# hszhao/semseg

Measured on NVIDIA H100. Metric: PSPNet50 473x473 training images/sec, higher is better.
Workload: dtype bf16

## Files before the change

include/semseg_b200.h:

```cpp
#ifndef SEMSEG_B200_H
#define SEMSEG_B200_H

#include <stdint.h>

#ifdef __cplusplus
extern "C" {
#endif

#define SEMSEG_OK 0
#define SEMSEG_E_INVALID (-1)
#define SEMSEG_E_CUDA (-2)
#define SEMSEG_E_UNSUPPORTED (-3)

#define SEMSEG_MAX_TAPS 9

const char* semseg_last_error(void);
int semseg_abi_version(void);
long long semseg_launch_count(void);

int semseg_psamask_fwd(int psa_type, const float* in, float* out, int N, int H, int W, int mH, int mW,
                       void* stream);
int semseg_psamask_bwd(int psa_type, const float* dout, float* din, int N, int H, int W, int mH, int mW,
                       void* stream);

// ... 46 lines not shown
  void* y_lo;
  const void* residual_lo;
  int32_t w_split;
  int32_t k_slices;
  int64_t slice_stride;
} semseg_conv_desc;

int semseg_conv_k_slices(int Cin, int taps, int max_kblocks);
int semseg_conv_splitk_rows(int M);
int semseg_conv_splitk_finish(const float* partial, int k_slices, long long slice_stride, int part_pitch, int M, int C,
                              int epi_mode, int relu, const float* scale, const float* shift, const void* residual,
                              const void* residual_lo, int res_pitch, void* y, void* y_lo, int y_pitch,
                              float* stats_partial, void* stream);
int semseg_conv_stats_rows(int N, int H, int W, int Cout);
int semseg_conv_fprop(const semseg_conv_desc* d, void* stream);

typedef struct semseg_wgrad_desc {
  int32_t N, H, W;
  int32_t Cin, Cout;
  const void* x;
  int32_t Nin, Hin, Win, x_pitch;
  const void* dy;
  int32_t dy_pitch;
  int32_t taps;
  int32_t dh[SEMSEG_MAX_TAPS], dw[SEMSEG_MAX_TAPS];
  int32_t img_mul, img_add[SEMSEG_MAX_TAPS];
  float* dw_partial;
  int32_t n_splits;
  const void* x_lo;
  const void* dy_lo;
} semseg_wgrad_desc;

int semseg_conv_wgrad_splits(const semseg_wgrad_desc* d);
int semseg_conv_wgrad(const semseg_wgrad_desc* d, void* stream);
int semseg_wgrad_reduce(const float* dw_partial, int n_splits, int taps, int Cout, int Cin, float* dw_oihw,
                        int accumulate, void* stream);

typedef struct semseg_pack_item {
  const float* w;
  void* wf;
  void* wd;
  void* wp;
  int Cout, Cin, taps;
  int cols_f, cols_d;
  int tile0, tiles_ci;
  int split;
} semseg_pack_item;
int semseg_pack_weights_multi(const semseg_pack_item* items_dev, int n_items, int n_tiles, int max_taps, void* stream);

// ... 267 lines not shown
```

semseg_b200/_lib.py:

```python
import ctypes
import os

_HERE = os.path.dirname(os.path.abspath(__file__))
LIB_PATH = os.path.join(_HERE, "lib", "libsemseg_b200.so")

MAX_TAPS = 9
EPI_RAW, EPI_AFFINE, EPI_F32 = 0, 1, 2
PSA_DENSE, PSA_NO_SOFTMAX = 1, 2

c_int = ctypes.c_int
c_i32 = ctypes.c_int32
c_vp = ctypes.c_void_p
c_f = ctypes.c_float
c_ll = ctypes.c_longlong
I9 = c_i32 * MAX_TAPS


class PackItem(ctypes.Structure):
    _fields_ = [
        ("w", c_vp), ("wf", c_vp), ("wd", c_vp), ("wp", c_vp),
        ("Cout", c_i32), ("Cin", c_i32), ("taps", c_i32),
        ("cols_f", c_i32), ("cols_d", c_i32),
        ("tile0", c_i32), ("tiles_ci", c_i32),
        ("split", c_i32),
# ... 72 lines not shown
    "semseg_psa_attend": (c_int, [c_int, c_int, c_vp, c_int, c_vp, c_vp, c_int, c_vp, c_vp, c_vp, c_int, c_int, c_int,
                                  c_int, c_int, c_int, c_int, c_f, c_vp]),
    "semseg_psa_attend_bwd_attn": (c_int, [c_int, c_vp, c_int, c_vp, c_vp, c_vp, c_int, c_vp, c_vp, c_int, c_vp, c_vp,
                                           c_int, c_vp, c_int, c_int, c_int, c_int, c_int, c_int, c_f, c_vp]),
    "semseg_psa_attend_ex": (c_int, [c_int, c_int, c_int, c_vp, c_int, c_vp, c_vp, c_int, c_vp, c_vp, c_vp, c_int,
                                     c_int, c_int, c_int, c_int, c_int, c_int, c_f, c_vp]),
    "semseg_psa_attend_bwd_attn_ex": (c_int, [c_int, c_int, c_vp, c_int, c_vp, c_vp, c_vp, c_int, c_vp, c_vp, c_int,
                                              c_vp, c_vp, c_int, c_vp, c_int, c_int, c_int, c_int, c_int, c_int, c_f,
                                              c_vp]),
    "semseg_conv_stats_rows": (c_int, [c_int, c_int, c_int, c_int]),
    "semseg_conv_k_slices": (c_int, [c_int, c_int, c_int]),
    "semseg_conv_splitk_rows": (c_int, [c_int]),
    "semseg_conv_splitk_finish": (c_int, [c_vp, c_int, c_ll, c_int, c_int, c_int, c_int, c_int, c_vp, c_vp, c_vp, c_vp,
                                          c_int, c_vp, c_vp, c_int, c_vp, c_vp]),
    "semseg_conv_fprop": (c_int, [ctypes.POINTER(ConvDesc), c_vp]),
    "semseg_conv_wgrad_splits": (c_int, [ctypes.POINTER(WgradDesc)]),
    "semseg_conv_wgrad": (c_int, [ctypes.POINTER(WgradDesc), c_vp]),
    "semseg_wgrad_reduce": (c_int, [c_vp, c_int, c_int, c_int, c_int, c_vp, c_int, c_vp]),
    "semseg_pack_weights_multi": (c_int, [c_vp, c_int, c_int, c_int, c_vp]),
    "semseg_sgd_chunk_elems": (c_int, []),
    "semseg_sgd_multi": (c_int, [c_vp, c_vp, c_int, c_int, ctypes.POINTER(SgdHyper), c_vp]),
    "semseg_ema_multi": (c_int, [c_vp, c_int, c_int, ctypes.c_double, c_vp]),
    "semseg_iou_hist": (c_int, [c_vp, c_vp, ctypes.c_longlong, c_int, ctypes.c_longlong, c_int, c_vp, c_vp]),
    "semseg_im2col3x3s2": (c_int, [c_vp, c_int, c_int, c_int, c_int, c_int, c_vp, c_vp]),
    "semseg_stem_dgrad3x3s2": (c_int, [c_vp, c_vp, c_int, c_int, c_int, c_int, c_int, c_int, c_int, c_int, c_vp, c_int,
                                       c_vp, c_vp]),
    "semseg_nchw_f32_to_nhwc_bf16": (c_int, [c_vp, c_vp, c_vp, c_int, c_int, c_int, c_int, c_int, c_vp]),
    "semseg_nhwc_bf16_to_nchw_f32": (c_int, [c_vp, c_vp, c_vp, c_int, c_int, c_int, c_int, c_int, c_vp]),
    "semseg_nhwc_f32_to_nchw_f32": (c_int, [c_vp, c_vp, c_int, c_int, c_int, c_int, c_int, c_vp]),
    "semseg_space_to_phases": (c_int, [c_vp, c_int, c_int, c_int, c_int, c_int, c_vp, c_vp]),
    "semseg_phases_to_space": (c_int, [c_vp, c_int, c_int, c_int, c_int, c_vp, c_vp]),
    "semseg_bn_merge_partials": (c_int, [c_vp, c_int, c_int, c_vp, c_vp]),
# ... 152 lines not shown
```

semseg_b200/csrc/conv_igemm.cu:

```cuda
#include "host_common.h"
#include "ptx.cuh"

namespace sb {

constexpr int kBlockM = 128;
constexpr int kBlockK = 64;
constexpr int kConvThreads = 384;
constexpr int kConsumerThreads = 256;
constexpr int kATileBytes = kBlockM * kBlockK * 2;
constexpr int kStageOutBytes = kBlockM * 64 * 2;
constexpr int kMiscBytes = 2048;

template <int BLOCK_N>
struct ConvCfg {
  static constexpr int kBTileBytes = BLOCK_N * kBlockK * 2;
  static constexpr int kStageBytes = kATileBytes + kBTileBytes;
  static constexpr int kStages = (BLOCK_N == 256) ? 4 : (BLOCK_N == 128 ? 6 : 8);
  static constexpr int kSmemBytes = kStages * kStageBytes + 2 * kStageOutBytes + kMiscBytes + 1024;
};

struct ConvKParams {
  int N, H, W;
  int Cin, Cout;
  int taps;
// ... 2 lines not shown
  int k_chunks;
  int dh[SEMSEG_MAX_TAPS], dw[SEMSEG_MAX_TAPS], wtap[SEMSEG_MAX_TAPS], img_add[SEMSEG_MAX_TAPS];
  int img_mul;
  int epi_mode, relu;
  const float* scale;
  const float* shift;
  const __nv_bfloat16* residual;
  const __nv_bfloat16* residual_lo;
  int res_pitch;
  int nseg;
  int k_slices, kb_per_slice;
  long long slice_stride;
  float* out_f32;
  int out_pitch;
  float* stats_partial;
};

template <int BLOCK_N, bool kSplit>
__global__ void __launch_bounds__(kConvThreads, 1)
conv_igemm_kernel(const __grid_constant__ CUtensorMap tmA, const __grid_constant__ CUtensorMap tmB,
                  const __grid_constant__ CUtensorMap tmC, const __grid_constant__ CUtensorMap tmA_lo,
                  const __grid_constant__ CUtensorMap tmB_lo, const __grid_constant__ CUtensorMap tmC_lo,
                  const ConvKParams p) {
  using Cfg = ConvCfg<BLOCK_N>;
  constexpr int kStages = Cfg::kStages;
  constexpr int kStageBytes = Cfg::kStageBytes;
  constexpr int kAcc = BLOCK_N / 2;
  const int num_items = p.num_m_tiles * p.n_tiles * p.k_slices;
  auto decode_item = [&](int item, int& m_tile, int& n_tile, int& k_slice) {
    k_slice = item % p.k_slices;
    item /= p.k_slices;
// ... 5 lines not shown
    const int tiles_per_img = p.tiles_h * p.tiles_w;
    img = m_tile / tiles_per_img;
    const int rem = m_tile - img * tiles_per_img;
    h0 = (rem / p.tiles_w) * p.bh;
    w0 = (rem % p.tiles_w) * p.bw;
  };

  extern __shared__ __align__(1024) uint8_t smem_raw[];
  uint8_t* smem = smem_raw + ((1024u - (smem_u32(smem_raw) & 1023u)) & 1023u);
  uint8_t* stage_base = smem;
  uint8_t* out_stage = smem + kStages * kStageBytes;
  uint8_t* misc = out_stage + 2 * kStageOutBytes;
  static_assert(kStages <= 16, "barrier area sized for <= 16 stages");
  uint64_t* full_bar = reinterpret_cast<uint64_t*>(misc);
  uint64_t* empty_bar = full_bar + 16;

  const int warp = threadIdx.x >> 5;
  const int lane = threadIdx.x & 31;
  const int nseg = kSplit ? p.nseg : 1;
  const int total_kblk = p.taps * p.k_chunks;
  auto slice_range = [&](int k_slice, int& kblk0, int& kblk1) {
    kblk0 = k_slice * p.kb_per_slice;
    kblk1 = min(kblk0 + p.kb_per_slice, total_kblk);
  };
  const uint32_t stage_tx = static_cast<uint32_t>(p.bh * p.bw) * 128u + static_cast<uint32_t>(Cfg::kBTileBytes);

  if (warp == 0 && lane == 0) {
    tma_prefetch_desc(&tmA);
    tma_prefetch_desc(&tmB);
    tma_prefetch_desc(&tmC);
    if (kSplit) {
      tma_prefetch_desc(&tmA_lo);
      tma_prefetch_desc(&tmB_lo);
      tma_prefetch_desc(&tmC_lo);
// ... 2 lines not shown
      mbar_init(&full_bar[i], 1);
      mbar_init(&empty_bar[i], kConsumerThreads);
    }
    fence_barrier_init();
  }
  if (p.stats_partial != nullptr) {
    float* row = p.stats_partial + static_cast<size_t>(blockIdx.x) * 4 * 3 * p.Cout;
    for (int i = threadIdx.x; i < 4 * 3 * p.Cout; i += kConvThreads) row[i] = 0.f;
  }
  __syncthreads();

  if (warp < 4) {
    setmaxnreg_dec<40>();
    if (warp == 0 && elect_one()) {
      int it = 0;
      for (int item = blockIdx.x; item < num_items; item += gridDim.x) {
        int m_tile, n_tile, k_slice, kblk0, kblk1;
        decode_item(item, m_tile, n_tile, k_slice);
        slice_range(k_slice, kblk0, kblk1);
        const int tiles_per_img = p.tiles_h * p.tiles_w;
        const int img = m_tile / tiles_per_img;
        const int rem = m_tile - img * tiles_per_img;
        const int h0 = (rem / p.tiles_w) * p.bh;
        const int w0 = (rem % p.tiles_w) * p.bw;
        const int n0 = n_tile * BLOCK_N;
        for (int kb = kblk0 * nseg; kb < kblk1 * nseg; ++kb, ++it) {
          const int s = it % kStages;
          const uint32_t par = (it / kStages) & 1;
          mbar_wait(&empty_bar[s], par ^ 1);
          const int ks = kb / nseg;
          const int seg = kb - ks * nseg;
          const int cb = ks / p.taps;
          const int t = ks - cb * p.taps;
          const CUtensorMap* mA = (kSplit && seg == 1) ? &tmA_lo : &tmA;
          const CUtensorMap* mB = (kSplit && seg == 2) ? &tmB_lo : &tmB;
          uint8_t* a_dst = stage_base + s * kStageBytes;
          uint8_t* b_dst = a_dst + kATileBytes;
          mbar_expect_tx(&full_bar[s], stage_tx);
          tma_load_4d(a_dst, mA, &full_bar[s], cb * kBlockK, w0 + p.dw[t], h0 + p.dh[t],
                      img * p.img_mul + p.img_add[t]);
          tma_load_3d(b_dst, mB, &full_bar[s], cb * kBlockK, n0, p.wtap[t]);
        }
      }
    }
  } else {
    setmaxnreg_inc<232>();
    const int ct = threadIdx.x - 128;
    const int wg = ct >> 7;
    const int wq = (ct >> 5) & 3;
    const int r_base = wg * 64 + wq * 16 + (lane >> 2);
    const int cq = 2 * (lane & 3);
    int it = 0;
    int store_buf = 0;
    float acc[kAcc];
    constexpr int kChunks = BLOCK_N / 64;
    const bool stats = p.stats_partial != nullptr && p.epi_mode == SEMSEG_EPI_RAW;
    float st_acc[kChunks][2], st_n = 0.f;
#pragma unroll
    for (int ch = 0; ch < kChunks; ++ch) st_acc[ch][0] = st_acc[ch][1] = 0.f;
    for (int item = blockIdx.x; item < num_items; item += gridDim.x) {
      int m_tile, n_tile, k_slice, kblk0, kblk1;
      decode_item(item, m_tile, n_tile, k_slice);
      slice_range(k_slice, kblk0, kblk1);
      const int num_kb = (kblk1 - kblk0) * nseg;
      if (p.epi_mode == SEMSEG_EPI_AFFINE && p.residual != nullptr && (lane & 3) < kChunks) {
        const int c = n_tile * BLOCK_N + 64 * (lane & 3);
        int img, h0, w0;
        tile_origin(m_tile, img, h0, w0);
#pragma unroll
        for (int i = 0; i < 2; ++i) {
          const int r = r_base + 8 * i, hi = r / p.bw, wi = r - hi * p.bw;
          if (c < p.Cout && r < p.bh * p.bw && h0 + hi < p.H && w0 + wi < p.W) {
            const long long ro = ((static_cast<long long>(img) * p.H + (h0 + hi)) * p.W + (w0 + wi)) * p.res_pitch + c;
            prefetch_l2(p.residual + ro);
            if (kSplit) prefetch_l2(p.residual_lo + ro);
// ... 169 lines not shown
            for (int v = 0; v < 3; ++v) old[ch][v] = st_dst[ch * 64 + v * p.Cout];
#pragma unroll
        for (int ch = 0; ch < kChunks; ++ch) {
          if (n0 + ch * 64 < p.Cout) {
            st_dst[ch * 64] = old[ch][0] + st_acc[ch][0];
            st_dst[ch * 64 + p.Cout] = old[ch][1] + st_acc[ch][1];
            st_dst[ch * 64 + 2 * p.Cout] = old[ch][2] + st_n;
          }
          st_acc[ch][0] = st_acc[ch][1] = 0.f;
        }
        st_n = 0.f;
      }
    }
    if (ct == 0) tma_store_wait_all<0>();
  }
}

static int conv_grid(int num_m_tiles, int n_tiles) {
  const int sms = num_sms();
  const long long tiles = static_cast<long long>(num_m_tiles) * n_tiles;
  return static_cast<int>(tiles < sms ? tiles : sms);
}

struct ConvMaps {
  CUtensorMap a, b, c, a_lo, b_lo, c_lo;
};

template <int BLOCK_N>
static int launch_conv(const ConvMaps& tm, const ConvKParams& kp, bool split, int grid, cudaStream_t stream) {
  using Cfg = ConvCfg<BLOCK_N>;
// ... 26 lines not shown

extern "C" int semseg_conv_k_slices(int Cin, int taps, int max_kblocks) {
  if (Cin <= 0 || taps <= 0 || max_kblocks <= 0) return SEMSEG_E_INVALID;
  const int total = taps * sb::cdiv(Cin, sb::kBlockK);
  const int per = sb::cdiv(total, sb::cdiv(total, max_kblocks));
  return sb::cdiv(total, per);
}

extern "C" int semseg_conv_stats_rows(int N, int H, int W, int Cout) {
  if (N <= 0 || H <= 0 || W <= 0 || Cout <= 0) return SEMSEG_E_INVALID;
  int bh, bw;
  sb::choose_box(H, W, sb::kBlockM, &bh, &bw);
  return 4 * sb::conv_grid(N * sb::cdiv(H, bh) * sb::cdiv(W, bw), sb::cdiv(Cout, conv_block_n(Cout)));
}

extern "C" int semseg_conv_fprop(const semseg_conv_desc* d, void* stream_) {
  using namespace sb;
  cudaStream_t stream = static_cast<cudaStream_t>(stream_);
  SB_CHECK_ARG(d != nullptr, "conv: null descriptor");
  SB_CHECK_ARG(d->N > 0 && d->H > 0 && d->W > 0 && d->Cin > 0 && d->Cout > 0, "conv: bad sizes");
  SB_CHECK_ARG(d->taps >= 1 && d->taps <= SEMSEG_MAX_TAPS, "conv: taps=%d out of range", d->taps);
  SB_CHECK_ARG(d->x && d->w, "conv: null x/w");
  SB_CHECK_ARG(d->x_pitch % 8 == 0 && d->x_pitch >= d->Cin, "conv: x_pitch %d must be a multiple of 8 and >= Cin",
               d->x_pitch);
  SB_CHECK_ARG(d->w_cols % 8 == 0 && d->w_cols >= d->Cin, "conv: w_cols %d must be a multiple of 8 and >= Cin",
               d->w_cols);
  SB_CHECK_ARG(d->epi_mode >= 0 && d->epi_mode <= 2, "conv: bad epi_mode");

  ConvKParams kp;
  memset(&kp, 0, sizeof(kp));
  kp.N = d->N; kp.H = d->H; kp.W = d->W; kp.Cin = d->Cin; kp.Cout = d->Cout; kp.taps = d->taps;
  choose_box(d->H, d->W, kBlockM, &kp.bh, &kp.bw);
  kp.tiles_h = cdiv(d->H, kp.bh);
// ... 8 lines not shown
  kp.epi_mode = d->epi_mode; kp.relu = d->relu;
  kp.scale = d->scale; kp.shift = d->shift;
  kp.residual = static_cast<const __nv_bfloat16*>(d->residual); kp.res_pitch = d->res_pitch;
  kp.residual_lo = static_cast<const __nv_bfloat16*>(d->residual_lo);
  const bool split = d->x_lo != nullptr;
  kp.nseg = split ? 3 : 1;
  if (split) {
    SB_CHECK_ARG(d->w_split != 0, "conv: split activations need split weights (w_split)");
    SB_CHECK_ARG(d->epi_mode == SEMSEG_EPI_F32 || d->y_lo != nullptr, "conv: split input needs a split output (y_lo)");
    SB_CHECK_ARG(!d->residual || d->residual_lo, "conv: split input needs a split residual (residual_lo)");
  } else {
    SB_CHECK_ARG(!d->y_lo && !d->residual_lo, "conv: lo planes given without x_lo");
  }
  kp.out_f32 = d->out_f32; kp.out_pitch = d->out_pitch;
  kp.stats_partial = d->stats_partial;

  const int block_n = conv_block_n(d->Cout);
  kp.n_tiles = cdiv(d->Cout, block_n);
  kp.k_slices = 1;
  kp.kb_per_slice = kp.taps * kp.k_chunks;
  kp.slice_stride = 0;
  if (d->k_slices > 1) {
    SB_CHECK_ARG(d->epi_mode == SEMSEG_EPI_F32, "conv: K slicing needs the F32 epilogue (partials are fp32)");
    SB_CHECK_ARG(d->slice_stride >= static_cast<long long>(d->N) * d->H * d->W * d->out_pitch,
                 "conv: slice_stride too small for an [N,H,W,out_pitch] partial");
    kp.kb_per_slice = cdiv(kp.taps * kp.k_chunks, d->k_slices);
    kp.k_slices = cdiv(kp.taps * kp.k_chunks, kp.kb_per_slice);
    SB_CHECK_ARG(kp.k_slices == d->k_slices, "conv: k_slices %d not realisable for %d K blocks (use %d)", d->k_slices,
                 kp.taps * kp.k_chunks, kp.k_slices);
    kp.slice_stride = d->slice_stride;
// ... 39 lines not shown
    uint64_t dims[4] = {(uint64_t)d->Cout, (uint64_t)d->W, (uint64_t)d->H, (uint64_t)d->N};
    uint64_t str[3] = {(uint64_t)d->y_pitch * 2, (uint64_t)d->y_pitch * 2 * d->W,
                       (uint64_t)d->y_pitch * 2 * d->W * d->H};
    uint32_t box[4] = {64u, (uint32_t)kp.bw, (uint32_t)kp.bh, 1};
    int r = encode_tmap_bf16(&tm.c, d->y, 4, dims, str, box);
    if (r) return r;
    tm.c_lo = tm.c;
    if (split && (r = encode_tmap_bf16(&tm.c_lo, d->y_lo, 4, dims, str, box))) return r;
  }
  switch (block_n) {
    case 256: return launch_conv<256>(tm, kp, split, grid, stream);
    case 128: return launch_conv<128>(tm, kp, split, grid, stream);
    default: return launch_conv<64>(tm, kp, split, grid, stream);
  }
}
```

semseg_b200/csrc/conv_wgrad.cu:

```cuda
#include "host_common.h"
#include "ptx.cuh"

namespace sb {

constexpr int kWgThreads = 384;
constexpr int kWgConsumerThreads = 256;
constexpr int kWgBoxPixels = 64;
constexpr int kWgBoxBytes = kWgBoxPixels * 128;
constexpr int kWgABoxes = 2;

template <int BN>
struct WgCfg {
  static constexpr int kBBoxes = BN / 64;
  static constexpr int kStageBytes = (kWgABoxes + kBBoxes) * kWgBoxBytes;
  static constexpr int kStages = BN == 256 ? 4 : (BN == 128 ? 6 : 8);
  static constexpr int kSmemBytes = kStages * kStageBytes + 1024 + 1024;
};

struct WgradKParams {
  int N, H, W, Cin, Cout, taps;
  int bh, bw, tiles_h, tiles_w, num_boxes;
  int co_tiles, ci_tiles, n_splits, boxes_per_split, block_n;
  int tu, cin_boxes, unit_taps, oob_img;
  int dh[SEMSEG_MAX_TAPS], dw[SEMSEG_MAX_TAPS], img_add[SEMSEG_MAX_TAPS];
// ... 293 lines not shown
    }
  }
  kp->boxes_per_split = cdiv(kp->num_boxes, splits);
  kp->n_splits = cdiv(kp->num_boxes, kp->boxes_per_split);
}

}

extern "C" int semseg_conv_wgrad_splits(const semseg_wgrad_desc* d) {
  if (!d || d->N <= 0 || d->H <= 0 || d->W <= 0 || d->Cin <= 0 || d->Cout <= 0) return SEMSEG_E_INVALID;
  sb::WgradKParams kp;
  sb::wgrad_geometry(d, &kp);
  return kp.n_splits;
}

extern "C" int semseg_conv_wgrad(const semseg_wgrad_desc* d, void* stream_) {
  using namespace sb;
  cudaStream_t stream = static_cast<cudaStream_t>(stream_);
  SB_CHECK_ARG(d != nullptr, "wgrad: null descriptor");
  SB_CHECK_ARG(d->N > 0 && d->H > 0 && d->W > 0 && d->Cin > 0 && d->Cout > 0, "wgrad: bad sizes");
  SB_CHECK_ARG(d->taps >= 1 && d->taps <= SEMSEG_MAX_TAPS, "wgrad: taps out of range");
  SB_CHECK_ARG(d->x && d->dy && d->dw_partial, "wgrad: null pointer");
  SB_CHECK_ARG(d->x_pitch % 8 == 0 && d->dy_pitch % 8 == 0, "wgrad: pitches must be multiples of 8");
  WgradKParams kp;
  memset(&kp, 0, sizeof(kp));
  wgrad_geometry(d, &kp);
  if (d->n_splits > 0)
    SB_CHECK_ARG(kp.n_splits == d->n_splits, "wgrad: n_splits %d not realisable (library would use %d)",
                 d->n_splits, kp.n_splits);
  for (int t = 0; t < d->taps; ++t) {
    kp.dh[t] = d->dh[t]; kp.dw[t] = d->dw[t]; kp.img_add[t] = d->img_add[t];
  }
  kp.img_mul = d->img_mul;
// ... 13 lines not shown
    tmDY_lo = tmDY;
    if (split && (r = encode_tmap_bf16(&tmDY_lo, d->dy_lo, 4, dims, str, box))) return r;
  }
  {
    uint64_t dims[4] = {(uint64_t)d->Cin, (uint64_t)d->Win, (uint64_t)d->Hin, (uint64_t)d->Nin};
    uint64_t str[3] = {(uint64_t)d->x_pitch * 2, (uint64_t)d->x_pitch * 2 * d->Win,
                       (uint64_t)d->x_pitch * 2 * d->Win * d->Hin};
    uint32_t box[4] = {64u, (uint32_t)kp.bw, (uint32_t)kp.bh, 1};
    int r = encode_tmap_bf16(&tmX, d->x, 4, dims, str, box);
    if (r) return r;
    tmX_lo = tmX;
    if (split && (r = encode_tmap_bf16(&tmX_lo, d->x_lo, 4, dims, str, box))) return r;
  }
  const int units = kp.unit_taps * kp.co_tiles * kp.ci_tiles * kp.n_splits;
  int rc = SEMSEG_OK;
  const int grid = units < num_sms() ? units : num_sms();
  switch (kp.block_n) {
    case 256: rc = launch_wgrad<256>(tmDY, tmX, tmDY_lo, tmX_lo, kp, grid, stream); break;
    case 128: rc = launch_wgrad<128>(tmDY, tmX, tmDY_lo, tmX_lo, kp, grid, stream); break;
    default: rc = launch_wgrad<64>(tmDY, tmX, tmDY_lo, tmX_lo, kp, grid, stream); break;
  }
  if (rc) return rc;
  SB_LAUNCHED();
  return SEMSEG_OK;
}

extern "C" int semseg_wgrad_reduce(const float* dw_partial, int n_splits, int taps, int Cout, int Cin,
                                   float* dw_oihw, int accumulate, void* stream_) {
  using namespace sb;
  cudaStream_t stream = static_cast<cudaStream_t>(stream_);
  SB_CHECK_ARG(dw_partial && dw_oihw && n_splits > 0 && taps > 0 && Cout > 0 && Cin > 0, "wgrad_reduce: bad args");
  SB_CHECK_ARG(taps <= kRedMaxTaps, "wgrad_reduce: at most 9 taps");
  const size_t plane = static_cast<size_t>(Cout) * Cin;
  const int groups = taps >= 8 ? 1 : 8 / taps;
  const dim3 block(32, taps, groups);
  if (plane % 4 == 0) {
    const size_t per_block = static_cast<size_t>(128) * groups;
    const unsigned blocks = static_cast<unsigned>((plane + per_block - 1) / per_block);
    const size_t smem = static_cast<size_t>(groups) * taps * (128 + 4) * sizeof(float);
// ... 11 lines not shown
```

semseg_b200/functional.py:

```python
import contextlib
import functools
import threading

import torch
import torch.distributed as dist
import torch.nn as nn
import torch.nn.functional as F

from . import losses
from . import ops
from . import p2p
from . import precision
from .dist_utils import gather_rank_stats
from .ops import EPI_RAW, EPI_AFFINE, EPI_F32


def packed(conv, need_dgrad=True, split=False):
    w = conv.weight
    key = (w._version, w.data_ptr(), need_dgrad, split)
    cache = conv.__dict__.get("_sb_pack")
    if cache is not None and cache[0] == key:
        return cache[1]
    if cache is not None and cache[0][:2] == key[:2] and cache[0][3] == split and cache[0][2]:
        return cache[1]
# ... 171 lines not shown
            raise NotImplementedError("semseg_b200: input gradient of a stride-2 conv needs Cin % 64 == 0")
        hh, wh = self.xin.shape[-3], self.xin.shape[-2]
        dxp = ops.empty_act((4 * n, hh, wh, pw.cin), ops.is_split(d_raw), d_raw.device)
        for q in range(4):
            sub = [t for t, a in zip(mirrored, self.img_add) if a == q * n]
            part = ops.act_batch_slice(dxp, q * n, (q + 1) * n)
            if sub:
                ops.conv_fprop(d_raw, pw.wd, pw.cin, sub, out=part, out_nhw=(n, hh, wh))
            else:
                part.zero_()
        dx = ops.phases_to_space(dxp, n, h, w)
        return dx if dx_add is None else ops.add_act(dx, dx_add)

    def wgrad(self, d_raw):
        pw = self.pw
        dw = ops.conv_wgrad(self.xin, d_raw, self.xin.shape[-1], pw.cout, self.taps, img_add=self.img_add)
        if self.kind == "patches":
            return dw[:, :9 * pw.cin, 0, 0].reshape(pw.cout, 3, 3, pw.cin).permute(0, 3, 1, 2).contiguous()
        return dw[:, :pw.cin].contiguous() if dw.shape[1] != pw.cin else dw


class _CbaState:
    __slots__ = ("form", "bn", "frozen", "relu", "has_res", "raw", "y", "mi", "ss", "pg")


def cba_forward(x, conv, bn, relu, residual, out=None, input_needs_grad=True, mode="batch"):
    form = _ConvForm(conv, x, input_needs_grad, mode)
    raw = mi = pg = None
    if mode == "batch":
        raw, sp = form.fprop(stats=True)
        pg = _sync_group(bn)
# ... 17 lines not shown
def cba_backward(st, dy, need_dx=True, need_dw=True, need_dres=False, dx_add=None, dx_nchw=False):
    bn = st.bn
    want_dres = st.has_res and need_dres
    if st.frozen:
        want_g, want_b = st.raw is not None, bn.bias is not None and bn.bias.requires_grad
        if not (need_dx or need_dw or want_dres or want_g or want_b):
            return None, None, None, None, None
        d_raw, dres, sums = ops.bn_bwd_frozen(dy if dy.is_contiguous() else dy.contiguous(), st.y, st.raw, bn.weight,
                                              bn.bias, bn.running_mean, bn.running_var, bn.eps, st.relu,
                                              want_dres=want_dres, want_sums=want_g or want_b)
        dgamma = sums[1] if want_g else None
        dbeta = sums[0] if want_b else None
    else:
        d_raw, dres, dgamma, dbeta = _bn_backward(st.pg, dy, st.y, st.raw, st.mi, bn.weight, st.relu, want_dres, st.ss)
    dx = st.form.dgrad(d_raw, dx_add, nchw=dx_nchw) if need_dx else None
    dw = st.form.wgrad(d_raw) if need_dw else None
    return dx, dw, dgamma, dbeta, dres


class _ConvBnAct(torch.autograd.Function):

    @staticmethod
    def forward(ctx, x, weight, gamma, beta, residual, conv, bn, relu, out, frozen):
        ctx.nchw = x.dtype != torch.bfloat16
        xa = ops.nchw_to_nhwc_bf16(x.contiguous().float(), split=precision.split_enabled()) if ctx.nchw else x
        y, st = cba_forward(xa, conv, bn, relu, residual, out, input_needs_grad=ctx.needs_input_grad[0],
                            mode="frozen" if frozen else "batch")
        ctx.st = st
        if out is not None:
            ctx.mark_dirty(out)
        return y
# ... 105 lines not shown
        ctx.save_for_backward(x)
        ctx.pw = pw
        return y

    @staticmethod
    def backward(ctx, dy):
        (x,) = ctx.saved_tensors
        pw = ctx.pw
        n, h, w, c = dy.shape
        cp = pw.wd.shape[-1]
        dyb = ops.f32_to_act(dy.contiguous(), ops.is_split(x))
        dx = dw = db = None
        if ctx.needs_input_grad[0]:
            dx, _ = ops.conv_fprop(dyb, pw.wd, pw.cin, ops.conv_taps(1, 1))
        if ctx.needs_input_grad[1]:
            dwp = ops.conv_wgrad(x, dyb, pw.cin, cp, ops.conv_taps(1, 1))
            dw = dwp[:c].contiguous()
        if ctx.needs_input_grad[2]:
            db = dy.sum(dim=(0, 1, 2))
        return dx, dw, db, None


def conv_bias_f32(x, conv):
    assert conv.kernel_size == (1, 1) and conv.stride == (1, 1) and x.shape[-1] % 8 == 0
    if torch.is_grad_enabled() and (x.requires_grad or conv.weight.requires_grad):
        return _ConvBiasF32.apply(x, conv.weight, conv.bias, conv)
    pw = packed(conv, need_dgrad=False, split=ops.is_split(x))
    y, _ = ops.conv_fprop(x, pw.wf, pw.cout, ops.conv_taps(1, 1), epi=EPI_F32, shift=conv.bias)
    return y


class _UpsampleCE(torch.autograd.Function):
# ... 524 lines not shown
```

semseg_b200/graphs.py:

```python
import os
import warnings

import torch
import torch.distributed as dist

from . import precision

WARMUP_CALLS = 3
MAX_GRAPHS = 4
_capturing = False
_boundary = None


def enabled():
    return os.environ.get("SEMSEG_B200_GRAPH", "1") != "0"


def capturing():
    return _capturing


def note_boundary(t):
    global _boundary
    if _capturing and t.requires_grad:
        _boundary = t
    return t


class _Step:
    __slots__ = ("key", "calls", "failed", "fwd", "bwd", "bwd2", "x", "y", "pred", "main", "aux", "g_main", "g_aux",
                 "grads", "grads2", "t_mid", "d_mid", "n_tail", "params", "pool", "keep", "launches", "dx_slot", "mix",
                 "mix_crit", "strong", "strong_crit", "fp", "fp_crit")

    def __init__(self, key):
# ... 117 lines not shown
    from . import _lib
    slots, seen = [], set()
    for mod in model.modules():
        for name, prm in mod._parameters.items():
            if prm is not None and prm.requires_grad and id(prm) not in seen:
                seen.add(id(prm))
                slots.append((mod, name, prm))
    st.params = [prm for _, _, prm in slots]
    st.x, st.y = torch.empty_like(x), torch.empty_like(y)
    st.x.copy_(x.detach())
    st.y.copy_(y)
    torch.cuda.synchronize()
    st.pool = torch.cuda.graph_pool_handle()
    st.fwd, st.bwd, st.bwd2 = torch.cuda.CUDAGraph(), torch.cuda.CUDAGraph(), None
    l0 = _lib.launch_count()
    global _boundary
    _capturing, _boundary = True, None
    proxies = []
    st.dx_slot = x.requires_grad
    x_in = st.x.detach().requires_grad_(True) if st.dx_slot else st.x
    x_leaf = [x_in] if st.dx_slot else []
    try:
        for mod, name, prm in slots:
            q = prm.detach().requires_grad_(True)
            mod._parameters[name] = q
            proxies.append(q)
        with torch.cuda.graph(st.fwd, pool=st.pool, capture_error_mode="thread_local"):
            with torch.enable_grad():
                st.pred, st.main, st.aux = impl(x_in, st.y)
        st.g_main, st.g_aux = torch.ones_like(st.main), torch.ones_like(st.aux)
        t_mid = _boundary
        head_ids = set()
        if t_mid is not None and os.environ.get("SEMSEG_B200_GRAPH_SEGMENTS", "2") != "1":
            for name in getattr(model, "_sb_head_modules", ()):
                head_ids.update(id(q) for q in getattr(model, name).parameters() if q.requires_grad)
        if head_ids:
            order = [k for k, q in enumerate(proxies) if id(q) in head_ids] + \
                    [k for k, q in enumerate(proxies) if id(q) not in head_ids]
            n_head = len(head_ids)
            st.params = [st.params[k] for k in order]
            prox_head = [proxies[k] for k in order[:n_head]]
            prox_tail = [proxies[k] for k in order[n_head:]]
            with torch.cuda.graph(st.bwd, pool=st.pool, capture_error_mode="thread_local"):
                gs = torch.autograd.grad((st.main, st.aux), [t_mid] + prox_tail, (st.g_main, st.g_aux), allow_unused=True)
            st.d_mid, st.grads = gs[0], gs[1:]
            st.bwd2 = torch.cuda.CUDAGraph()
            with torch.cuda.graph(st.bwd2, pool=st.pool, capture_error_mode="thread_local"):
                st.grads2 = torch.autograd.grad((t_mid,), prox_head + x_leaf, (st.d_mid,), allow_unused=True)
            st.t_mid, st.n_tail = t_mid.detach(), len(prox_tail)
        else:
            with torch.cuda.graph(st.bwd, pool=st.pool, capture_error_mode="thread_local"):
                st.grads = torch.autograd.grad((st.main, st.aux), proxies + x_leaf, (st.g_main, st.g_aux),
                                               allow_unused=True)
    finally:
        _capturing, _boundary = False, None
        for mod, name, prm in slots:
            mod._parameters[name] = prm
    st.launches = _lib.launch_count() - l0
    crit = getattr(model, "criterion", None)
    if getattr(crit, "_mix_state", None) is not None:
        st.mix, st.mix_crit = crit._mix_state, crit
    if getattr(crit, "strong", None) is not None:
        st.strong, st.strong_crit = crit._strong_state, crit
    if getattr(crit, "fp_weight", 0.0) > 0.0:
        st.fp, st.fp_crit = crit._fp_state, crit
    st.pred, st.main, st.aux = st.pred.detach(), st.main.detach(), st.aux.detach()
    del proxies, x_in, x_leaf
    st.keep = model.__dict__.get("_sb_pack_plan")
    teacher = _teacher(getattr(model, "criterion", None))
    if teacher is not None:
# ... 77 lines not shown
```

semseg_b200/ops.py:

```python
import ctypes

import torch

from . import _lib
from . import p2p
from ._lib import ConvDesc, WgradDesc, EPI_RAW, EPI_AFFINE, EPI_F32, MAX_TAPS


X3_MAX_KBLOCKS = 8

_raw_stream = getattr(torch._C, "_cuda_getCurrentRawStream", None)
_cur_device = getattr(torch._C, "_cuda_getDevice", None)


def _stream():
    if _raw_stream is not None and _cur_device is not None:
        return ctypes.c_void_p(_raw_stream(_cur_device()))
    return ctypes.c_void_p(torch.cuda.current_stream().cuda_stream)


def _ptr(t):
    return ctypes.c_void_p(t.data_ptr()) if t is not None else ctypes.c_void_p(0)


def _require_cuda(*ts):
    for t in ts:
        if t is not None and not t.is_cuda:
            raise _lib.SemsegError("semseg_b200 ops require CUDA tensors (no CPU fallback); got device %s" % t.device)


def is_split(t):
    return t is not None and t.dim() == 5

# ... 278 lines not shown
    if shift is not None:
        assert shift.dtype == torch.float32 and shift.numel() >= cout
        d.shift = shift.data_ptr()
    if residual is not None:
        rn, rh, rw, rc, rp = _nhwc_meta(residual)
        assert (rn, rh, rw, rc) == (n, h, w, cout) and is_split(residual) == split
        d.residual, d.res_pitch, d.residual_lo = residual.data_ptr(), rp, _lo_int(residual)
    k_slices = int(lib.semseg_conv_k_slices(cin, len(taps), X3_MAX_KBLOCKS)) if (split and epi != EPI_F32) else 1
    if k_slices > 1:
        part = torch.empty((k_slices, n, h, w, cout), dtype=torch.float32, device=x.device)
        d.epi_mode, d.relu = EPI_F32, 0
        d.out_f32, d.out_pitch = part.data_ptr(), cout
        d.k_slices, d.slice_stride = k_slices, part.stride(0)
        sc, sh, rs, rsl, rpitch, ylo = d.scale, d.shift, d.residual, d.residual_lo, d.res_pitch, d.y_lo
        d.scale = d.shift = d.residual = d.residual_lo = d.y_lo = None
        _lib.check(lib.semseg_conv_fprop(ctypes.byref(d), _stream()), "semseg_conv_fprop (K-sliced)")
        m = n * h * w
        if stats:
            assert epi == EPI_RAW
            sp = torch.empty((int(lib.semseg_conv_splitk_rows(m)), 3, cout), dtype=torch.float32, device=x.device)
        _lib.check(lib.semseg_conv_splitk_finish(_ptr(part), k_slices, part.stride(0), cout, m, cout, epi,
                                                 int(bool(relu)), sc, sh, rs, rsl, rpitch, d.y, ylo, d.y_pitch,
                                                 _ptr(sp), _stream()), "semseg_conv_splitk_finish")
        return y, sp
    if stats:
        assert epi == EPI_RAW
        sp = torch.empty((conv_stats_rows(n, h, w, cout), 3, cout), dtype=torch.float32, device=x.device)
        d.stats_partial = sp.data_ptr()
    _lib.check(lib.semseg_conv_fprop(ctypes.byref(d), _stream()), "semseg_conv_fprop")
    return y, sp


def conv_wgrad(x, dy, cin, cout, taps, grad_out=None, accumulate=False, img_add=None):
    _require_cuda(x, dy)
    lib = _lib.load()
    nin, hin, win, xc, xp = _nhwc_meta(x)
    n, h, w, dc, dp = _nhwc_meta(dy)
    assert xc >= cin and dc >= cout
    assert img_add is not None or (nin, hin, win) == (n, h, w)
    _same_form(x, dy)
    d = WgradDesc()
    d.N, d.H, d.W, d.Cin, d.Cout = n, h, w, cin, cout
    d.x, d.Nin, d.Hin, d.Win, d.x_pitch = x.data_ptr(), nin, hin, win, xp
    d.dy, d.dy_pitch = dy.data_ptr(), dp
    d.x_lo, d.dy_lo = _lo_int(x), _lo_int(dy)
    _fill_taps(d, taps, with_wtap=False, img_add=img_add)
    d.n_splits = 0
    splits = lib.semseg_conv_wgrad_splits(ctypes.byref(d))
    if splits <= 0:
        raise _lib.SemsegError("semseg_conv_wgrad_splits failed (%d)" % splits)
    ntaps = len(taps)
    part = torch.empty((splits, ntaps, cout, cin), dtype=torch.float32, device=x.device)
    d.dw_partial = part.data_ptr()
    d.n_splits = splits
    _lib.check(lib.semseg_conv_wgrad(ctypes.byref(d), _stream()), "semseg_conv_wgrad")
    k = int(round(ntaps ** 0.5))
    if grad_out is None:
        grad_out = torch.empty((cout, cin, k, k), dtype=torch.float32, device=x.device)
        accumulate = False
    assert grad_out.is_contiguous() and grad_out.dtype == torch.float32
    _lib.check(lib.semseg_wgrad_reduce(_ptr(part), splits, ntaps, cout, cin, _ptr(grad_out), int(accumulate),
                                       _stream()), "semseg_wgrad_reduce")
    return grad_out


def nchw_to_nhwc_bf16(x, pad_to=8, split=False):
    _require_cuda(x)
    lib = _lib.load()
    assert x.dtype == torch.float32 and x.is_contiguous()
    n, c, h, w = x.shape
# ... 872 lines not shown
```

Before: 299.7.

## Overlap weight-gradient convs on a side stream with dynamically scheduled convs

During CUDA-graph capture, weight-gradient convolutions are launched on a side stream with their grid capped to leave SMs free, so they can run concurrently with the data-gradient path on the main stream. The conv fprop kernel gains an optional dynamic tile scheduler. A global atomic counter per stream slot hands out work items, and the producer forwards each item ID to the consumers through shared memory, so CTAs that share the GPU with side-stream work balance their load. This adds atomic traffic, a self-resetting counter that assumes no two concurrent launches share a slot, and stream synchronisation joins at the end of backward.

```diff
diff --git a/include/semseg_b200.h b/include/semseg_b200.h
--- a/include/semseg_b200.h
+++ b/include/semseg_b200.h
@@ -84,6 +84,8 @@
                               float* stats_partial, void* stream);
 int semseg_conv_stats_rows(int N, int H, int W, int Cout);
 int semseg_conv_fprop(const semseg_conv_desc* d, void* stream);
+int semseg_conv_sched_slots(void);
+int semseg_conv_fprop_sched(const semseg_conv_desc* d, int slot, void* stream);
 
 typedef struct semseg_wgrad_desc {
   int32_t N, H, W;
@@ -103,6 +105,7 @@
 
 int semseg_conv_wgrad_splits(const semseg_wgrad_desc* d);
 int semseg_conv_wgrad(const semseg_wgrad_desc* d, void* stream);
+int semseg_conv_wgrad_grid(const semseg_wgrad_desc* d, int max_ctas, void* stream);
 int semseg_wgrad_reduce(const float* dw_partial, int n_splits, int taps, int Cout, int Cin, float* dw_oihw,
                         int accumulate, void* stream);
 
diff --git a/semseg_b200/_lib.py b/semseg_b200/_lib.py
--- a/semseg_b200/_lib.py
+++ b/semseg_b200/_lib.py
@@ -110,8 +110,11 @@
     "semseg_conv_splitk_finish": (c_int, [c_vp, c_int, c_ll, c_int, c_int, c_int, c_int, c_int, c_vp, c_vp, c_vp, c_vp,
                                           c_int, c_vp, c_vp, c_int, c_vp, c_vp]),
     "semseg_conv_fprop": (c_int, [ctypes.POINTER(ConvDesc), c_vp]),
+    "semseg_conv_sched_slots": (c_int, []),
+    "semseg_conv_fprop_sched": (c_int, [ctypes.POINTER(ConvDesc), c_int, c_vp]),
     "semseg_conv_wgrad_splits": (c_int, [ctypes.POINTER(WgradDesc)]),
     "semseg_conv_wgrad": (c_int, [ctypes.POINTER(WgradDesc), c_vp]),
+    "semseg_conv_wgrad_grid": (c_int, [ctypes.POINTER(WgradDesc), c_int, c_vp]),
     "semseg_wgrad_reduce": (c_int, [c_vp, c_int, c_int, c_int, c_int, c_vp, c_int, c_vp]),
     "semseg_pack_weights_multi": (c_int, [c_vp, c_int, c_int, c_int, c_vp]),
     "semseg_sgd_chunk_elems": (c_int, []),
diff --git a/semseg_b200/csrc/conv_igemm.cu b/semseg_b200/csrc/conv_igemm.cu
--- a/semseg_b200/csrc/conv_igemm.cu
+++ b/semseg_b200/csrc/conv_igemm.cu
@@ -40,7 +40,11 @@
   float* out_f32;
   int out_pitch;
   float* stats_partial;
+  unsigned* sched;
 };
+
+constexpr int kSchedSlots = 64;
+__device__ unsigned g_conv_sched[kSchedSlots][2];
 
 template <int BLOCK_N, bool kSplit>
 __global__ void __launch_bounds__(kConvThreads, 1)
@@ -76,10 +80,12 @@
   static_assert(kStages <= 16, "barrier area sized for <= 16 stages");
   uint64_t* full_bar = reinterpret_cast<uint64_t*>(misc);
   uint64_t* empty_bar = full_bar + 16;
+  int* stage_item = reinterpret_cast<int*>(empty_bar + 16);
 
   const int warp = threadIdx.x >> 5;
   const int lane = threadIdx.x & 31;
   const int nseg = kSplit ? p.nseg : 1;
+  const bool dynamic = p.sched != nullptr;
   const int total_kblk = p.taps * p.k_chunks;
   auto slice_range = [&](int k_slice, int& kblk0, int& kblk1) {
     kblk0 = k_slice * p.kb_per_slice;
@@ -112,7 +118,9 @@
     setmaxnreg_dec<40>();
     if (warp == 0 && elect_one()) {
       int it = 0;
-      for (int item = blockIdx.x; item < num_items; item += gridDim.x) {
+      for (int item = dynamic ? static_cast<int>(atomicAdd(&p.sched[0], 1u)) : static_cast<int>(blockIdx.x), next;
+           item < num_items; item = next) {
+        next = dynamic ? static_cast<int>(atomicAdd(&p.sched[0], 1u)) : item + static_cast<int>(gridDim.x);
         int m_tile, n_tile, k_slice, kblk0, kblk1;
         decode_item(item, m_tile, n_tile, k_slice);
         slice_range(k_slice, kblk0, kblk1);
@@ -134,11 +142,18 @@
           const CUtensorMap* mB = (kSplit && seg == 2) ? &tmB_lo : &tmB;
           uint8_t* a_dst = stage_base + s * kStageBytes;
           uint8_t* b_dst = a_dst + kATileBytes;
+          if (dynamic && kb == kblk0 * nseg) stage_item[s] = item;
           mbar_expect_tx(&full_bar[s], stage_tx);
           tma_load_4d(a_dst, mA, &full_bar[s], cb * kBlockK, w0 + p.dw[t], h0 + p.dh[t],
                       img * p.img_mul + p.img_add[t]);
           tma_load_3d(b_dst, mB, &full_bar[s], cb * kBlockK, n0, p.wtap[t]);
         }
+      }
+      if (dynamic) {
+        const int s = it % kStages;
+        mbar_wait(&empty_bar[s], ((it / kStages) & 1) ^ 1);
+        stage_item[s] = num_items;
+        mbar_arrive(&full_bar[s]);
       }
     }
   } else {
@@ -156,7 +171,13 @@
     float st_acc[kChunks][2], st_n = 0.f;
 #pragma unroll
     for (int ch = 0; ch < kChunks; ++ch) st_acc[ch][0] = st_acc[ch][1] = 0.f;
-    for (int item = blockIdx.x; item < num_items; item += gridDim.x) {
+    for (int item = static_cast<int>(blockIdx.x);; item += gridDim.x) {
+      if (dynamic) {
+        const int s = it % kStages;
+        mbar_wait(&full_bar[s], (it / kStages) & 1);
+        item = stage_item[s];
+      }
+      if (item >= num_items) break;
       int m_tile, n_tile, k_slice, kblk0, kblk1;
       decode_item(item, m_tile, n_tile, k_slice);
       slice_range(k_slice, kblk0, kblk1);
@@ -356,6 +377,16 @@
     }
     if (ct == 0) tma_store_wait_all<0>();
   }
+  if (dynamic) {
+    __syncthreads();
+    if (threadIdx.x == 0) {
+      __threadfence();
+      if (atomicAdd(&p.sched[1], 1u) == gridDim.x - 1) {
+        atomicExch(&p.sched[0], 0u);
+        atomicExch(&p.sched[1], 0u);
+      }
+    }
+  }
 }
 
 static int conv_grid(int num_m_tiles, int n_tiles) {
@@ -412,9 +443,10 @@
   return 4 * sb::conv_grid(N * sb::cdiv(H, bh) * sb::cdiv(W, bw), sb::cdiv(Cout, conv_block_n(Cout)));
 }
 
-extern "C" int semseg_conv_fprop(const semseg_conv_desc* d, void* stream_) {
+extern "C" int semseg_conv_sched_slots() { return sb::kSchedSlots; }
+
+static int conv_fprop_launch(const semseg_conv_desc* d, int slot, cudaStream_t stream) {
   using namespace sb;
-  cudaStream_t stream = static_cast<cudaStream_t>(stream_);
   SB_CHECK_ARG(d != nullptr, "conv: null descriptor");
   SB_CHECK_ARG(d->N > 0 && d->H > 0 && d->W > 0 && d->Cin > 0 && d->Cout > 0, "conv: bad sizes");
   SB_CHECK_ARG(d->taps >= 1 && d->taps <= SEMSEG_MAX_TAPS, "conv: taps=%d out of range", d->taps);
@@ -453,6 +485,21 @@
   }
   kp.out_f32 = d->out_f32; kp.out_pitch = d->out_pitch;
   kp.stats_partial = d->stats_partial;
+  kp.sched = nullptr;
+  if (slot >= 0) {
+    SB_CHECK_ARG(d->stats_partial == nullptr, "conv_fprop_sched: a launch with statistics needs the static order");
+    static std::atomic<unsigned*> sched_base[64];
+    int dev = 0;
+    SB_CUDA(cudaGetDevice(&dev));
+    unsigned* base = dev >= 0 && dev < 64 ? sched_base[dev].load(std::memory_order_acquire) : nullptr;
+    if (base == nullptr) {
+      void* b = nullptr;
+      SB_CUDA(cudaGetSymbolAddress(&b, g_conv_sched));
+      base = static_cast<unsigned*>(b);
+      if (dev >= 0 && dev < 64) sched_base[dev].store(base, std::memory_order_release);
+    }
+    kp.sched = base + 2 * slot;
+  }
 
   const int block_n = conv_block_n(d->Cout);
   kp.n_tiles = cdiv(d->Cout, block_n);
@@ -522,3 +569,13 @@
     default: return launch_conv<64>(tm, kp, split, grid, stream);
   }
 }
+
+extern "C" int semseg_conv_fprop(const semseg_conv_desc* d, void* stream) {
+  return conv_fprop_launch(d, -1, static_cast<cudaStream_t>(stream));
+}
+
+extern "C" int semseg_conv_fprop_sched(const semseg_conv_desc* d, int slot, void* stream) {
+  SB_CHECK_ARG(slot >= 0 && slot < sb::kSchedSlots, "conv_fprop_sched: slot %d out of range [0, %d)", slot,
+               sb::kSchedSlots);
+  return conv_fprop_launch(d, slot, static_cast<cudaStream_t>(stream));
+}
diff --git a/semseg_b200/csrc/conv_wgrad.cu b/semseg_b200/csrc/conv_wgrad.cu
--- a/semseg_b200/csrc/conv_wgrad.cu
+++ b/semseg_b200/csrc/conv_wgrad.cu
@@ -331,9 +331,8 @@
   return kp.n_splits;
 }
 
-extern "C" int semseg_conv_wgrad(const semseg_wgrad_desc* d, void* stream_) {
+static int conv_wgrad_launch(const semseg_wgrad_desc* d, int max_ctas, cudaStream_t stream) {
   using namespace sb;
-  cudaStream_t stream = static_cast<cudaStream_t>(stream_);
   SB_CHECK_ARG(d != nullptr, "wgrad: null descriptor");
   SB_CHECK_ARG(d->N > 0 && d->H > 0 && d->W > 0 && d->Cin > 0 && d->Cout > 0, "wgrad: bad sizes");
   SB_CHECK_ARG(d->taps >= 1 && d->taps <= SEMSEG_MAX_TAPS, "wgrad: taps out of range");
@@ -377,7 +376,8 @@
   }
   const int units = kp.unit_taps * kp.co_tiles * kp.ci_tiles * kp.n_splits;
   int rc = SEMSEG_OK;
-  const int grid = units < num_sms() ? units : num_sms();
+  int grid = units < num_sms() ? units : num_sms();
+  if (max_ctas > 0 && grid > max_ctas) grid = max_ctas;
   switch (kp.block_n) {
     case 256: rc = launch_wgrad<256>(tmDY, tmX, tmDY_lo, tmX_lo, kp, grid, stream); break;
     case 128: rc = launch_wgrad<128>(tmDY, tmX, tmDY_lo, tmX_lo, kp, grid, stream); break;
@@ -386,6 +386,15 @@
   if (rc) return rc;
   SB_LAUNCHED();
   return SEMSEG_OK;
+}
+
+extern "C" int semseg_conv_wgrad(const semseg_wgrad_desc* d, void* stream) {
+  return conv_wgrad_launch(d, 0, static_cast<cudaStream_t>(stream));
+}
+
+extern "C" int semseg_conv_wgrad_grid(const semseg_wgrad_desc* d, int max_ctas, void* stream) {
+  SB_CHECK_ARG(max_ctas >= 1, "wgrad_grid: max_ctas %d must be >= 1", max_ctas);
+  return conv_wgrad_launch(d, max_ctas, static_cast<cudaStream_t>(stream));
 }
 
 extern "C" int semseg_wgrad_reduce(const float* dw_partial, int n_splits, int taps, int Cout, int Cin,
diff --git a/semseg_b200/functional.py b/semseg_b200/functional.py
--- a/semseg_b200/functional.py
+++ b/semseg_b200/functional.py
@@ -7,6 +7,7 @@
 import torch.nn as nn
 import torch.nn.functional as F
 
+from . import graphs
 from . import losses
 from . import ops
 from . import p2p
@@ -209,7 +210,8 @@
 
     def wgrad(self, d_raw):
         pw = self.pw
-        dw = ops.conv_wgrad(self.xin, d_raw, self.xin.shape[-1], pw.cout, self.taps, img_add=self.img_add)
+        dw = ops.conv_wgrad(self.xin, d_raw, self.xin.shape[-1], pw.cout, self.taps, img_add=self.img_add,
+                            max_ctas=graphs.wgrad_max_ctas())
         if self.kind == "patches":
             return dw[:, :9 * pw.cin, 0, 0].reshape(pw.cout, 3, 3, pw.cin).permute(0, 3, 1, 2).contiguous()
         return dw[:, :pw.cin].contiguous() if dw.shape[1] != pw.cin else dw
@@ -257,7 +259,7 @@
     else:
         d_raw, dres, dgamma, dbeta = _bn_backward(st.pg, dy, st.y, st.raw, st.mi, bn.weight, st.relu, want_dres, st.ss)
     dx = st.form.dgrad(d_raw, dx_add, nchw=dx_nchw) if need_dx else None
-    dw = st.form.wgrad(d_raw) if need_dw else None
+    dw = graphs.beside(lambda: st.form.wgrad(d_raw), d_raw, st.form.xin) if need_dw else None
     return dx, dw, dgamma, dbeta, dres
 
 
@@ -393,8 +395,8 @@
         if ctx.needs_input_grad[0]:
             dx, _ = ops.conv_fprop(dyb, pw.wd, pw.cin, ops.conv_taps(1, 1))
         if ctx.needs_input_grad[1]:
-            dwp = ops.conv_wgrad(x, dyb, pw.cin, cp, ops.conv_taps(1, 1))
-            dw = dwp[:c].contiguous()
+            dw = graphs.beside(lambda: ops.conv_wgrad(x, dyb, pw.cin, cp, ops.conv_taps(1, 1),
+                                                      max_ctas=graphs.wgrad_max_ctas())[:c].contiguous(), x, dyb)
         if ctx.needs_input_grad[2]:
             db = dy.sum(dim=(0, 1, 2))
         return dx, dw, db, None
diff --git a/semseg_b200/graphs.py b/semseg_b200/graphs.py
--- a/semseg_b200/graphs.py
+++ b/semseg_b200/graphs.py
@@ -10,6 +10,10 @@
 MAX_GRAPHS = 4
 _capturing = False
 _boundary = None
+WGRAD_RESERVE_SMS = 32
+WGRAD_BESIDE = True
+_side = {}
+_side_keep = []
 
 
 def enabled():
@@ -18,6 +22,38 @@
 
 def capturing():
     return _capturing
+
+
+def _side_stream(device):
+    s = _side.get(device)
+    if s is None:
+        s = _side[device] = torch.cuda.Stream(device=device)
+    return s
+
+
+def beside(fn, *keep):
+    if not (_capturing and WGRAD_BESIDE) or precision.split_enabled():
+        return fn()
+    cur = torch.cuda.current_stream()
+    side = _side_stream(cur.device.index)
+    side.wait_stream(cur)
+    with torch.cuda.stream(side):
+        out = fn()
+    _side_keep.append((keep, out))
+    return out
+
+
+def wgrad_max_ctas():
+    if not (_capturing and WGRAD_BESIDE) or precision.split_enabled():
+        return 0
+    sms = torch.cuda.get_device_properties(torch.cuda.current_device()).multi_processor_count
+    return max(1, sms - WGRAD_RESERVE_SMS)
+
+
+def _join_side():
+    if _side_keep:
+        torch.cuda.current_stream().wait_stream(_side[torch.cuda.current_device()])
+    _side_keep.clear()
 
 
 def note_boundary(t):
@@ -165,6 +201,7 @@
     st.pool = torch.cuda.graph_pool_handle()
     st.fwd, st.bwd, st.bwd2 = torch.cuda.CUDAGraph(), torch.cuda.CUDAGraph(), None
     l0 = _lib.launch_count()
+    _side_stream(torch.cuda.current_device())
     global _boundary
     _capturing, _boundary = True, None
     proxies = []
@@ -194,17 +231,21 @@
             prox_tail = [proxies[k] for k in order[n_head:]]
             with torch.cuda.graph(st.bwd, pool=st.pool, capture_error_mode="thread_local"):
                 gs = torch.autograd.grad((st.main, st.aux), [t_mid] + prox_tail, (st.g_main, st.g_aux), allow_unused=True)
+                _join_side()
             st.d_mid, st.grads = gs[0], gs[1:]
             st.bwd2 = torch.cuda.CUDAGraph()
             with torch.cuda.graph(st.bwd2, pool=st.pool, capture_error_mode="thread_local"):
                 st.grads2 = torch.autograd.grad((t_mid,), prox_head + x_leaf, (st.d_mid,), allow_unused=True)
+                _join_side()
             st.t_mid, st.n_tail = t_mid.detach(), len(prox_tail)
         else:
             with torch.cuda.graph(st.bwd, pool=st.pool, capture_error_mode="thread_local"):
                 st.grads = torch.autograd.grad((st.main, st.aux), proxies + x_leaf, (st.g_main, st.g_aux),
                                                allow_unused=True)
+                _join_side()
     finally:
         _capturing, _boundary = False, None
+        _side_keep.clear()
         for mod, name, prm in slots:
             mod._parameters[name] = prm
     st.launches = _lib.launch_count() - l0
diff --git a/semseg_b200/ops.py b/semseg_b200/ops.py
--- a/semseg_b200/ops.py
+++ b/semseg_b200/ops.py
@@ -17,6 +17,29 @@
     if _raw_stream is not None and _cur_device is not None:
         return ctypes.c_void_p(_raw_stream(_cur_device()))
     return ctypes.c_void_p(torch.cuda.current_stream().cuda_stream)
+
+
+_sched_slots = {}
+SCHED_SPLIT = False
+
+
+def _sched_slot(stream):
+    dev = _cur_device() if _cur_device is not None else torch.cuda.current_device()
+    key = (dev, stream.value)
+    slot = _sched_slots.get(key)
+    if slot is None:
+        used = sum(1 for k in _sched_slots if k[0] == dev)
+        slot = _sched_slots[key] = used if used < _lib.load().semseg_conv_sched_slots() else -1
+    return slot
+
+
+def _conv_launch(lib, d, what):
+    stream = _stream()
+    slot = _sched_slot(stream) if not d.stats_partial and (SCHED_SPLIT or not d.x_lo) else -1
+    if slot >= 0:
+        _lib.check(lib.semseg_conv_fprop_sched(ctypes.byref(d), slot, stream), what)
+    else:
+        _lib.check(lib.semseg_conv_fprop(ctypes.byref(d), stream), what)
 
 
 def _ptr(t):
@@ -325,7 +348,7 @@
         d.k_slices, d.slice_stride = k_slices, part.stride(0)
         sc, sh, rs, rsl, rpitch, ylo = d.scale, d.shift, d.residual, d.residual_lo, d.res_pitch, d.y_lo
         d.scale = d.shift = d.residual = d.residual_lo = d.y_lo = None
-        _lib.check(lib.semseg_conv_fprop(ctypes.byref(d), _stream()), "semseg_conv_fprop (K-sliced)")
+        _conv_launch(lib, d, "semseg_conv_fprop (K-sliced)")
         m = n * h * w
         if stats:
             assert epi == EPI_RAW
@@ -338,11 +361,11 @@
         assert epi == EPI_RAW
         sp = torch.empty((conv_stats_rows(n, h, w, cout), 3, cout), dtype=torch.float32, device=x.device)
         d.stats_partial = sp.data_ptr()
-    _lib.check(lib.semseg_conv_fprop(ctypes.byref(d), _stream()), "semseg_conv_fprop")
+    _conv_launch(lib, d, "semseg_conv_fprop")
     return y, sp
 
 
-def conv_wgrad(x, dy, cin, cout, taps, grad_out=None, accumulate=False, img_add=None):
+def conv_wgrad(x, dy, cin, cout, taps, grad_out=None, accumulate=False, img_add=None, max_ctas=0):
     _require_cuda(x, dy)
     lib = _lib.load()
     nin, hin, win, xc, xp = _nhwc_meta(x)
@@ -364,7 +387,10 @@
     part = torch.empty((splits, ntaps, cout, cin), dtype=torch.float32, device=x.device)
     d.dw_partial = part.data_ptr()
     d.n_splits = splits
-    _lib.check(lib.semseg_conv_wgrad(ctypes.byref(d), _stream()), "semseg_conv_wgrad")
+    if max_ctas > 0:
+        _lib.check(lib.semseg_conv_wgrad_grid(ctypes.byref(d), int(max_ctas), _stream()), "semseg_conv_wgrad_grid")
+    else:
+        _lib.check(lib.semseg_conv_wgrad(ctypes.byref(d), _stream()), "semseg_conv_wgrad")
     k = int(round(ntaps ** 0.5))
     if grad_out is None:
         grad_out = torch.empty((cout, cin, k, k), dtype=torch.float32, device=x.device)
```

Measured after the change: 305.3, median of 6. 1.9% higher.
